# jojolebarjos/board-game-simulator-python

Measured on AMD Instinct MI355X. Metric: env-steps/sec, Connect4(6,7,4) random rollout, batch=2^20 per GPU, higher is better.
Workload: dtype u64

## Files before the change

### board-game-simulator-python_amd/csrc/connect_kernels.hip

```cpp
#include <type_traits>

#include "bgs_common.h"
#include "bgs_internal.h"
#include "connect_board.h"

#ifndef BGS_TU_ID
#define BGS_TU_ID "unknown"
#endif
extern "C" const char bgs_tu_id_connect[] = BGS_TU_ID;

namespace bgs {
namespace {

template <int NW_, int SH, int SW, int SK>
struct Geo {
    static constexpr int NW = NW_;
    static constexpr int STATIC_H = SH, STATIC_W = SW, STATIC_K = SK;
    static constexpr int MAXW = SW ? SW : BGS_CONNECT_MAX_W;
    int rh, rw, rk;
    __device__ __forceinline__ int h() const { return SH ? SH : rh; }
    __device__ __forceinline__ int w() const { return SW ? SW : rw; }
    __device__ __forceinline__ int k() const { return SK ? SK : rk; }
    __device__ __forceinline__ uint32_t all_columns() const { return (1u << w()) - 1u; }
};
// ... 733 lines not shown
        skip = 0;

        if (was_live != 0 && live == 0) {
            const uint32_t code = st ? st : (open == 0u ? BGS_ST_DRAW : BGS_ST_RUNNING);
            *reinterpret_cast<uint64_t*>(reinterpret_cast<char*>(plane0) + (game * 8u)) = p[0];
            *reinterpret_cast<uint64_t*>(reinterpret_cast<char*>(plane1) + (game * 8u)) = p[1];
            *(reinterpret_cast<uint8_t*>(status_out) + game) = (uint8_t)code;
            *reinterpret_cast<uint16_t*>(reinterpret_cast<char*>(reward_out) + (game * 2u)) = reward_pair(code);
            if (CODES) codes.add(game, code);
        }
    } while (__builtin_amdgcn_ballot_w64(live != 0) || taken < avail);
    if (CODES) codes.flush(codes_out, begin);
    add_steps(steps, stepped);
}

template <class G, int OPEN_BLOCKS, bool PER_PLY = false>
struct OpenedWords {
    static constexpr int LAST = G::STATIC_H > 0 ? (G::STATIC_H * G::STATIC_W + 3) / 4 - 1 : 11;
    static constexpr int COUNT = PER_PLY ? 1 : (LAST - OPEN_BLOCKS + 1 > 1 ? LAST - OPEN_BLOCKS + 1 : 1);
    static constexpr int QUADS = (COUNT + 3) / 4;
    static_assert(LAST <= 11 && OPEN_BLOCKS >= 1 && OPEN_BLOCKS <= 4, "three philox calls cover blocks 0 .. 11");
};

template <int QUADS>
struct OpenedPool {
    static constexpr uint32_t SLOTS = 64;
    uint64_t plane[2][SLOTS];
    uint32_t cols[SLOTS];
    uint4 words[QUADS][SLOTS];
};

constexpr uint32_t kReplayMark = 1u << 28;
constexpr uint32_t kReplayRow = 0x80000000u;

template <class G, int OPEN_BLOCKS, bool PER_PLY>
constexpr bool deferred_opening() {
    if constexpr (G::STATIC_H > 0 && G::STATIC_W > 0 && G::STATIC_K > 0)
        return !PER_PLY && kDeferredOpeningStages > 0 && OPEN_BLOCKS == kRolloutOpeningBlocks && kRolloutOpeningBlocks == 3 &&
               deferred_opening_ok(G::STATIC_H, G::STATIC_W, G::STATIC_K);
    else
        return false;
}

template <class G, class Pool>
__device__ __forceinline__ void open_games_deferred(const G& g, Pool& pool, uint32_t slot, uint64_t seed, uint64_t id, bool mine) {
    constexpr uint32_t ONES = 0x11111111u;
    const uint32_t top = (uint32_t)g.h() + 7u;
    const uint32_t columns = ONES & ((1u << (4 * g.w())) - 1u);
    const uint32_t stride = (uint32_t)g.h() + 1u;
    uint64_t q[2] = {0, 0};
    uint32_t h4 = top * columns;
    auto cheap_ply = [&](uint32_t j, uint32_t draw, bool wrap) {
        const uint32_t col = sample_index(draw, (uint32_t)g.w());
        const uint32_t sh = col * 4u;
        const uint32_t v = (h4 >> sh) & 15u;
        uint32_t pos = col * stride + top - v;
        if (wrap) pos &= 63u;
        q[j & 1u] |= 1ull << pos;
        h4 -= 1u << sh;
    };
    auto blind_block = [&](uint32_t word, bool wrap) -> bool {
        cheap_ply(0u, sub_draw<0>(word), wrap);
        cheap_ply(1u, sub_draw<1>(word), wrap);
        cheap_ply(2u, sub_draw<2>(word), wrap);
        const bool closed = ((h4 >> 3) & ONES) != columns;
        cheap_ply(3u, sub_draw<3>(word), wrap);
        return closed;
    };
    auto park = [&](uint32_t cols, const uint4& lo, const uint4& hi) {
        pool.plane[0][slot] = q[0];
        pool.plane[1][slot] = q[1];
        pool.cols[slot] = cols;
        pool.words[0][slot] = lo;
        pool.words[1][slot] = hi;
    };
    const Philox4 a = philox4x32_10(seed, id, 0u);
    cheap_ply(0u, sub_draw<0>(a.v[0]), false);
    cheap_ply(1u, sub_draw<1>(a.v[0]), false);
    cheap_ply(2u, sub_draw<2>(a.v[0]), false);
    cheap_ply(3u, sub_draw<3>(a.v[0]), false);
    uint32_t* const slot_words0 = reinterpret_cast<uint32_t*>(&pool.words[0][slot]);
    uint32_t* const slot_words1 = reinterpret_cast<uint32_t*>(&pool.words[1][slot]);
    slot_words0[0] = a.v[1]; slot_words0[1] = a.v[2]; slot_words0[2] = a.v[3];
    uint64_t id_after = id;
    asm volatile("" : "+v"(id_after) : : "memory");
    uint32_t word9, word10;
    {
        Philox4 c = philox4x32_10(seed, id_after, 2u);
        slot_words1[3] = c.v[0];
        word9 = c.v[1];
        word10 = c.v[2];
        asm volatile("" : "+v"(id_after), "+v"(word9), "+v"(word10) : : "memory");
    }
    {
        const Philox4 b = philox4x32_10(seed, id_after, 1u);
        slot_words0[3] = b.v[0];
        slot_words1[0] = b.v[1]; slot_words1[1] = b.v[2]; slot_words1[2] = b.v[3];
    }
    pool.plane[0][slot] = q[0];
    pool.plane[1][slot] = q[1];
    pool.cols[slot] = mine ? (h4 | kReplayMark) : 0u;
    asm volatile("" ::: "memory");
    blind_block(slot_words0[0], false);
    const bool closed = blind_block(slot_words0[1], false);
    const uint32_t hits = four_in_a_row_low_hits(q[0], g.h()) | four_in_a_row_low_hits(q[1], g.h());
    const bool clean = mine && !closed && hits == 0u;
    if (clean) {
        const uint4 lo = pool.words[0][slot], hi = pool.words[1][slot];
        park(h4, make_uint4(lo.z, lo.w, hi.x, hi.y), make_uint4(hi.z, hi.w, word9, word10));
    }
    if constexpr (kDeferredOpeningStages >= 2) {
        asm volatile("" ::: "memory");
        const bool closed2 = blind_block(slot_words0[0], true);
        const uint32_t hits2 = four_in_a_row_low_hits(q[0], g.h()) | four_in_a_row_low_hits(q[1], g.h());
        if (clean && !closed2 && hits2 == 0u) {
            const uint4 lo = pool.words[0][slot], hi = pool.words[1][slot];
            park(h4, make_uint4(lo.y, lo.z, lo.w, hi.x), make_uint4(hi.y, hi.z, hi.w, 0u));
        }
    }
}

template <class G, int OPEN_BLOCKS, bool CODES, bool PER_PLY>
__global__ void __launch_bounds__(BGS_BLOCK)
k_connect_rollout_opened(G g, uint64_t* __restrict__ planes, uint8_t* __restrict__ status, uint16_t* __restrict__ reward,
                         int64_t n, uint64_t seed, uint64_t first_game, unsigned long long* __restrict__ steps,
                         uint32_t games_per_wave, uint32_t* __restrict__ codes_out) {
    using OW = OpenedWords<G, OPEN_BLOCKS, PER_PLY>;
    constexpr int NWORDS = OW::QUADS * 4;
    using Pool = OpenedPool<OW::QUADS>;
    constexpr bool DEFER = deferred_opening<G, OPEN_BLOCKS, PER_PLY>();
    static_assert(!DEFER || NWORDS == 8, "a replayed game refills rows 5 .. 7 with the words of blocks 8 .. 10");
    extern __shared__ uint32_t code_lds[];
    __shared__ Pool pools[BGS_BLOCK / BGS_WAVE];
    __shared__ uint32_t lane_words[BGS_BLOCK / BGS_WAVE][NWORDS][BGS_WAVE];
    constexpr uint32_t ONES = 0x11111111u;
    const uint32_t top = (uint32_t)g.h() + 7u;
    const uint32_t columns = g.w() >= 8 ? ONES : (ONES & ((1u << (4 * g.w())) - 1u));
    const uint32_t stride = (uint32_t)g.h() + 1u;
    const uint32_t column_top = 8u * columns;
    const uint64_t eights = 0x88888888ull;

    const uint32_t wave = __builtin_amdgcn_readfirstlane(blockIdx.x * (BGS_BLOCK / BGS_WAVE) + (threadIdx.x >> 6));
    const uint32_t lane = threadIdx.x & 63u;
    const int64_t begin = (int64_t)wave * games_per_wave;
    const int64_t end = begin + games_per_wave < n ? begin + games_per_wave : n;
    const uint32_t avail = begin < end ? (uint32_t)(end - begin) : 0u;
    uint32_t taken = 0;
    uint32_t opened = 0;
    uint64_t* __restrict__ const plane0 = planes + begin;
    uint64_t* __restrict__ const plane1 = planes + n + begin;
    Pool& pool = pools[threadIdx.x >> 6];

    uint64_t p[2] = {0, 0};
    uint32_t hts = 0, live = 0, game = 0, stepped = 0;
    bool anywon = false;
    uint32_t wnext = 0;
    uint32_t* const my_words = &lane_words[threadIdx.x >> 6][0][lane];
    uint32_t wrow = 0;
    uint32_t myblk = 0;

    if (avail == 0u) return;
    uint8_t* const outcome = reinterpret_cast<uint8_t*>(code_lds + (threadIdx.x >> 6) * (games_per_wave >> 2));
    for (uint32_t i = lane; i < ((avail + 3u) >> 2); i += BGS_WAVE) reinterpret_cast<uint32_t*>(outcome)[i] = 0u;
    __builtin_amdgcn_wave_barrier();

    auto full_ply = [&](auto j_tag, uint32_t draw, uint64_t (&q)[2], uint32_t& h4, uint32_t& op, uint32_t& alive,
                        bool& won_any) {
        constexpr uint32_t J = decltype(j_tag)::value;
        const uint32_t cnt = (uint32_t)__popc(op);
        const uint32_t idx = sample_index(draw, cnt);
        uint64_t cmp64;
        {
            uint64_t carry;
            asm("v_mad_u64_u32 %0, %1, %2, %3, %4" : "=v"(cmp64), "=s"(carry) : "v"(idx - op), "s"(ONES), "v"(eights));
        }
        const uint32_t cmp = (uint32_t)cmp64;
        uint32_t col = (uint32_t)__popc(cmp & column_top);
        if (g.w() >= 8) col &= 7u;
        const uint32_t sh = col * 4u;
        const uint32_t v = (h4 >> sh) & 15u;
        uint32_t base = col * stride + top;
        asm("" : "+v"(base));
        uint32_t pos = base - v;
        if ((uint32_t)g.w() * stride + top > 63u) pos &= 63u;
        const uint32_t act = alive;
        uint64_t& mine = q[J & 1u];
        const uint64_t bit = 1ull << pos;
        mine = ((uint64_t)and_or((uint32_t)(bit >> 32), act, (uint32_t)(mine >> 32)) << 32) |
               and_or((uint32_t)bit, act, (uint32_t)mine);
        h4 += act << sh;
        op = (h4 >> 3) & ONES;
        bool won;
        if (g.k() == 4) {
            won = ply_run_of_four(g, mine, pos);
        } else {
            Bits<1> b;
            b.w[0] = mine;
            won = has_run(g, b);
        }
        won_any = won_any || won;
        alive = (won || op == 0u) ? 0u : alive;
    };
    auto outcome_of = [&](const uint64_t (&q)[2], bool won_any) -> uint32_t {
        const uint32_t stones = (uint32_t)__popcll(q[0]) + (uint32_t)__popcll(q[1]);
        stepped += stones;
        return won_any ? ((stones - 1u) & 1u) + 1u : (uint32_t)BGS_ST_DRAW;
    };
    auto cheap_ply = [&](uint32_t j, uint32_t draw, uint64_t (&q)[2], uint32_t& h4) {
        const uint32_t col = sample_index(draw, (uint32_t)g.w());
        const uint32_t sh = col * 4u;
        const uint32_t v = (h4 >> sh) & 15u;
        const uint32_t pos = col * stride + top - v;
        q[j & 1u] |= 1ull << pos;
        h4 -= 1u << sh;
    };
    auto refetch = [&](uint64_t lane_seed, uint64_t id) {
        if (wrow == (kReplayRow | 7u)) {
            if (live != 0u) {
                const Philox4 d = philox4x32_10(lane_seed, id, 2u);
                my_words[5 * BGS_WAVE] = d.v[0];
                my_words[6 * BGS_WAVE] = d.v[1];
                my_words[7 * BGS_WAVE] = d.v[2];
            }
            wrow = 5u;
        }
    };
    auto play_block = [&]() {
        const uint32_t was_live = live;
        Philox4 four = {{0u, 0u, 0u, 0u}};
        uint32_t word = 0u;
        if constexpr (PER_PLY) {
            four = philox4x32_10(seed, first_game + (uint64_t)(begin + game), myblk);
            myblk += 1u;
        } else if constexpr (DEFER) {
            word = wnext;
            if (__builtin_amdgcn_ballot_w64(wrow == (kReplayRow | 7u))) refetch(seed, first_game + (uint64_t)(begin + game));
            wnext = my_words[wrow * BGS_WAVE];
            const int32_t up = (int32_t)(wrow + 1u);
            wrow = (uint32_t)(up < NWORDS - 1 ? up : NWORDS - 1);
        } else {
            word = wnext;
            wnext = my_words[wrow * BGS_WAVE];
            wrow = wrow + 1u < (uint32_t)NWORDS - 1u ? wrow + 1u : (uint32_t)NWORDS - 1u;
        }
        uint32_t open = (hts >> 3) & ONES;
        full_ply(std::integral_constant<uint32_t, 0>{}, PER_PLY ? four.v[0] : sub_draw<0>(word), p, hts, open, live, anywon);
        full_ply(std::integral_constant<uint32_t, 1>{}, PER_PLY ? four.v[1] : sub_draw<1>(word), p, hts, open, live, anywon);
        full_ply(std::integral_constant<uint32_t, 2>{}, PER_PLY ? four.v[2] : sub_draw<2>(word), p, hts, open, live, anywon);
        full_ply(std::integral_constant<uint32_t, 3>{}, PER_PLY ? four.v[3] : sub_draw<3>(word), p, hts, open, live, anywon);
        if (was_live != 0 && live == 0) {
            *reinterpret_cast<uint64_t*>(reinterpret_cast<char*>(plane0) + (game * 8u)) = p[0];
            *reinterpret_cast<uint64_t*>(reinterpret_cast<char*>(plane1) + (game * 8u)) = p[1];
            outcome[game] = (uint8_t)outcome_of(p, anywon);
        }
    };
    auto take = [&](uint32_t which) {
        game = which;
        const uint32_t slot = which & (Pool::SLOTS - 1u);
        p[0] = pool.plane[0][slot];
        p[1] = pool.plane[1][slot];
        hts = pool.cols[slot];
        if constexpr (PER_PLY) {
            myblk = (uint32_t)OPEN_BLOCKS;
        } else {
#pragma unroll
            for (int k = 0; k < OW::QUADS; ++k) {
                const uint4 v = pool.words[k][slot];
                if (k == 0) wnext = v.x; else my_words[(4 * k) * BGS_WAVE] = v.x;
                my_words[(4 * k + 1) * BGS_WAVE] = v.y;
                my_words[(4 * k + 2) * BGS_WAVE] = v.z;
                my_words[(4 * k + 3) * BGS_WAVE] = v.w;
            }
        }
        wrow = DEFER ? 1u | ((hts << 3) & kReplayRow) : 1u;
        anywon = false;
        live = hts != 0u ? ~0u : 0u;
    };
    auto open_games = [&]() {
        const uint32_t og = opened + lane;
        const uint64_t id = first_game + (uint64_t)(begin + og);
        if constexpr (DEFER) {
            open_games_deferred(g, pool, og & (Pool::SLOTS - 1u), seed, id, og < avail);
            opened += 64u;
            return;
        }
        uint64_t q[2] = {0, 0};
        uint32_t h4 = top * columns, alive = ~0u, op = columns;
        bool won_any = false;
        uint32_t words[12];
        Philox4 own = philox4x32_10(seed, id, 0u);
        using J0 = std::integral_constant<uint32_t, 0>; using J1 = std::integral_constant<uint32_t, 1>;
        using J2 = std::integral_constant<uint32_t, 2>; using J3 = std::integral_constant<uint32_t, 3>;
#define BGS_DRAW_OF(JT, b) (PER_PLY ? own.v[JT::value] : sub_draw<JT::value>(words[b]))
        if constexpr (!PER_PLY) {
            words[0] = own.v[0]; words[1] = own.v[1]; words[2] = own.v[2]; words[3] = own.v[3];
#pragma unroll
            for (int c = 1; c < 3; ++c) {
                if (4 * c <= OW::LAST) {
                    const Philox4 d = philox4x32_10(seed, id, (uint32_t)c);
                    words[4 * c] = d.v[0]; words[4 * c + 1] = d.v[1]; words[4 * c + 2] = d.v[2]; words[4 * c + 3] = d.v[3];
                } else {
                    words[4 * c] = words[4 * c + 1] = words[4 * c + 2] = words[4 * c + 3] = 0u;
                }
            }
        } else {
#pragma unroll
            for (int c = 0; c < 12; ++c) words[c] = 0u;
        }
        cheap_ply(0u, BGS_DRAW_OF(J0, 0), q, h4);
        cheap_ply(1u, BGS_DRAW_OF(J1, 0), q, h4);
        cheap_ply(2u, BGS_DRAW_OF(J2, 0), q, h4);
        cheap_ply(3u, BGS_DRAW_OF(J3, 0), q, h4);
        if (OPEN_BLOCKS >= 2) {
            if constexpr (PER_PLY) own = philox4x32_10(seed, id, 1u);
            cheap_ply(0u, BGS_DRAW_OF(J0, 1), q, h4);
            cheap_ply(1u, BGS_DRAW_OF(J1, 1), q, h4);
            op = (h4 >> 3) & ONES;
            full_ply(J2{}, BGS_DRAW_OF(J2, 1), q, h4, op, alive, won_any);
            full_ply(J3{}, BGS_DRAW_OF(J3, 1), q, h4, op, alive, won_any);
        }
#pragma unroll
        for (int ob = 2; ob < OPEN_BLOCKS; ++ob) {
            if constexpr (PER_PLY) own = philox4x32_10(seed, id, (uint32_t)ob);
            full_ply(J0{}, BGS_DRAW_OF(J0, ob), q, h4, op, alive, won_any);
            full_ply(J1{}, BGS_DRAW_OF(J1, ob), q, h4, op, alive, won_any);
            full_ply(J2{}, BGS_DRAW_OF(J2, ob), q, h4, op, alive, won_any);
            full_ply(J3{}, BGS_DRAW_OF(J3, ob), q, h4, op, alive, won_any);
        }
#undef BGS_DRAW_OF
        if (OPEN_BLOCKS >= 2 && og < avail && alive == 0) {
            plane0[og] = q[0];
            plane1[og] = q[1];
            outcome[og] = (uint8_t)outcome_of(q, won_any);
        }
        const uint32_t slot = og & (Pool::SLOTS - 1u);
        pool.plane[0][slot] = q[0];
        pool.plane[1][slot] = q[1];
        pool.cols[slot] = alive ? h4 : 0u;
#pragma unroll
        for (int k = 0; k < OW::QUADS; ++k) {
            auto at = [&](int i) { return OPEN_BLOCKS + i <= 11 ? words[OPEN_BLOCKS + i <= 11 ? OPEN_BLOCKS + i : 11] : 0u; };
            pool.words[k][slot] = make_uint4(at(4 * k), at(4 * k + 1), at(4 * k + 2), at(4 * k + 3));
        }
        opened += 64u;
    };

    while (taken < avail) {
        const uint64_t need = __builtin_amdgcn_ballot_w64(live == 0);
        if (need) {
            const uint32_t wanted = (uint32_t)__popcll(need);
            const uint32_t rank = __builtin_amdgcn_mbcnt_hi((uint32_t)(need >> 32), __builtin_amdgcn_mbcnt_lo((uint32_t)need, 0u));
            const uint32_t have = opened - taken;
            if (wanted > have && opened < avail) {
                const bool first = live == 0 && rank < have;
                const bool second = live == 0 && !first;
                if (first && taken + rank < avail) take(taken + rank);
                __builtin_amdgcn_fence(__ATOMIC_ACQ_REL, "wavefront");
                __builtin_amdgcn_wave_barrier();
                open_games();
                __builtin_amdgcn_fence(__ATOMIC_ACQ_REL, "wavefront");
                __builtin_amdgcn_wave_barrier();
                if (second && taken + rank < avail) take(taken + rank);
            } else if (live == 0 && taken + rank < avail) {
                take(taken + rank);
            }
            taken = avail - taken < wanted ? avail : taken + wanted;
        }
        play_block();
    }
    while (__builtin_amdgcn_ballot_w64(live != 0)) play_block();

    __builtin_amdgcn_fence(__ATOMIC_ACQ_REL, "wavefront");
    __builtin_amdgcn_wave_barrier();
    uint8_t* __restrict__ const status_out = status + begin;
    uint16_t* __restrict__ const reward_out = reward + begin;
    uint8_t* __restrict__ const packed_out = reinterpret_cast<uint8_t*>(codes_out) + (begin >> 2);
    for (uint32_t g4 = lane * 4u; g4 < avail; g4 += BGS_WAVE * 4u) {
        const uint32_t four = reinterpret_cast<const uint32_t*>(outcome)[g4 >> 2];
        if (CODES) packed_out[g4 >> 2] = (uint8_t)((four & 3u) | ((four >> 6) & 0xCu) | ((four >> 12) & 0x30u) | ((four >> 18) & 0xC0u));
        if (g4 + 4u <= avail) {
            *reinterpret_cast<uint32_t*>(status_out + g4) = four;
            uint2 r;
            r.x = (uint32_t)reward_pair(four & 255u) | ((uint32_t)reward_pair((four >> 8) & 255u) << 16);
            r.y = (uint32_t)reward_pair((four >> 16) & 255u) | ((uint32_t)reward_pair(four >> 24) << 16);
            *reinterpret_cast<uint2*>(reward_out + g4) = r;
        } else {
            for (uint32_t k = 0; g4 + k < avail; ++k) {
                const uint32_t ck = (four >> (8u * k)) & 255u;
                status_out[g4 + k] = (uint8_t)ck;
                reward_out[g4 + k] = reward_pair(ck);
            }
        }
    }
    add_steps(steps, stepped);
}

template <class G, int OPEN_BLOCKS, bool CODES>
__global__ void __launch_bounds__(BGS_BLOCK)
k_connect_rollout_opened_steps(G g, const ConnectGroup tab, int64_t n, uint32_t games_per_wave) {
    using OW = OpenedWords<G, OPEN_BLOCKS, false>;
    constexpr int NWORDS = OW::QUADS * 4;
    using Pool = OpenedPool<OW::QUADS>;
    constexpr bool DEFER = deferred_opening<G, OPEN_BLOCKS, false>();
    static_assert(!DEFER || NWORDS == 8, "a replayed game refills rows 5 .. 7 with the words of blocks 8 .. 10");
    extern __shared__ uint32_t code_lds[];
    __shared__ Pool pools[BGS_BLOCK / BGS_WAVE];
    __shared__ uint32_t lane_words[BGS_BLOCK / BGS_WAVE][NWORDS][BGS_WAVE];
    constexpr uint32_t ONES = 0x11111111u;
    const uint32_t top = (uint32_t)g.h() + 7u;
    const uint32_t columns = g.w() >= 8 ? ONES : (ONES & ((1u << (4 * g.w())) - 1u));
    const uint32_t stride = (uint32_t)g.h() + 1u;
    const uint32_t column_top = 8u * columns;
    const uint64_t eights = 0x88888888ull;

    const uint32_t wave = __builtin_amdgcn_readfirstlane(blockIdx.x * (BGS_BLOCK / BGS_WAVE) + (threadIdx.x >> 6));
    const uint32_t lane = threadIdx.x & 63u;
    const int64_t begin = (int64_t)wave * games_per_wave;
    const int64_t end = begin + games_per_wave < n ? begin + games_per_wave : n;
    const uint32_t avail = begin < end ? (uint32_t)(end - begin) : 0u;
    const uint32_t nsteps = (uint32_t)tab.count;
    uint32_t taken = 0, opened = 0;
    Pool& pool = pools[threadIdx.x >> 6];

    uint32_t cur = 0;
    bool pending = false;
    uint64_t cur_seed = tab.step[0].seed, cur_first = tab.step[0].first_game;
    uint64_t* cur_planes = tab.step[0].planes ? tab.step[0].planes + begin : nullptr;
    uint64_t* prev_planes = nullptr;
    uint64_t prev_seed = 0, prev_first = 0;

    uint64_t p[2] = {0, 0};
    uint32_t hts = 0, live = 0, game = 0;
    uint32_t old = 0;
    uint32_t stepped0 = 0, stepped1 = 0;
    bool anywon = false;
    uint32_t wnext = 0;
    uint32_t* const my_words = &lane_words[threadIdx.x >> 6][0][lane];
    uint32_t wrow = 0;

    if (avail == 0u) return;
    uint8_t* const slices = reinterpret_cast<uint8_t*>(code_lds + (threadIdx.x >> 6) * (games_per_wave >> 1));
    auto slice_of = [&](uint32_t s) { return slices + (s & 1u) * games_per_wave; };
    auto zero_slice = [&](uint32_t s) {
        uint32_t* const w = reinterpret_cast<uint32_t*>(slice_of(s));
        for (uint32_t i = lane; i < ((avail + 3u) >> 2); i += BGS_WAVE) w[i] = 0u;
        __builtin_amdgcn_fence(__ATOMIC_ACQ_REL, "wavefront");
        __builtin_amdgcn_wave_barrier();
    };
    zero_slice(0u);

    auto full_ply = [&](auto j_tag, uint32_t draw, uint64_t (&q)[2], uint32_t& h4, uint32_t& op, uint32_t& alive,
                        bool& won_any) {
        constexpr uint32_t J = decltype(j_tag)::value;
        const uint32_t cnt = (uint32_t)__popc(op);
        const uint32_t idx = sample_index(draw, cnt);
        uint64_t cmp64;
        {
            uint64_t carry;
            asm("v_mad_u64_u32 %0, %1, %2, %3, %4" : "=v"(cmp64), "=s"(carry) : "v"(idx - op), "s"(ONES), "v"(eights));
        }
        const uint32_t cmp = (uint32_t)cmp64;
        uint32_t col = (uint32_t)__popc(cmp & column_top);
        if (g.w() >= 8) col &= 7u;
        const uint32_t sh = col * 4u;
        const uint32_t v = (h4 >> sh) & 15u;
        uint32_t base = col * stride + top;
        asm("" : "+v"(base));
        uint32_t pos = base - v;
        if ((uint32_t)g.w() * stride + top > 63u) pos &= 63u;
        const uint32_t act = alive;
        uint64_t& mine = q[J & 1u];
        const uint64_t bit = 1ull << pos;
        mine = ((uint64_t)and_or((uint32_t)(bit >> 32), act, (uint32_t)(mine >> 32)) << 32) |
               and_or((uint32_t)bit, act, (uint32_t)mine);
        h4 += act << sh;
        op = (h4 >> 3) & ONES;
        bool won;
        if (g.k() == 4) {
            won = ply_run_of_four(g, mine, pos);
        } else {
            Bits<1> b;
            b.w[0] = mine;
            won = has_run(g, b);
        }
        won_any = won_any || won;
        alive = (won || op == 0u) ? 0u : alive;
    };
    auto outcome_of = [&](const uint64_t (&q)[2], bool won_any, uint32_t parity) -> uint32_t {
        const uint32_t stones = (uint32_t)__popcll(q[0]) + (uint32_t)__popcll(q[1]);
        stepped0 += parity ? 0u : stones;
        stepped1 += parity ? stones : 0u;
        return won_any ? ((stones - 1u) & 1u) + 1u : (uint32_t)BGS_ST_DRAW;
    };
    auto cheap_ply = [&](uint32_t j, uint32_t draw, uint64_t (&q)[2], uint32_t& h4) {
        const uint32_t col = sample_index(draw, (uint32_t)g.w());
        const uint32_t sh = col * 4u;
        const uint32_t v = (h4 >> sh) & 15u;
        const uint32_t pos = col * stride + top - v;
        q[j & 1u] |= 1ull << pos;
        h4 -= 1u << sh;
    };
    auto refetch = [&]() {
        const bool at = wrow == (kReplayRow | 7u);
#pragma unroll
        for (uint32_t o = 0; o < 2u; ++o) {
            const bool here = at && live != 0u && old == o;
            if (__builtin_amdgcn_ballot_w64(here) == 0) continue;
            if (here) {
                const Philox4 d = philox4x32_10(o ? prev_seed : cur_seed, (o ? prev_first : cur_first) + (uint64_t)(begin + game), 2u);
                my_words[5 * BGS_WAVE] = d.v[0];
                my_words[6 * BGS_WAVE] = d.v[1];
                my_words[7 * BGS_WAVE] = d.v[2];
            }
        }
        if (at) wrow = 5u;
    };
    auto play_block = [&]() {
        const uint32_t was_live = live;
        const uint32_t word = wnext;
        if constexpr (DEFER) {
            if (__builtin_amdgcn_ballot_w64(wrow == (kReplayRow | 7u))) refetch();
            wnext = my_words[wrow * BGS_WAVE];
            const int32_t up = (int32_t)(wrow + 1u);
            wrow = (uint32_t)(up < NWORDS - 1 ? up : NWORDS - 1);
        } else {
            wnext = my_words[wrow * BGS_WAVE];
            wrow = wrow + 1u < (uint32_t)NWORDS - 1u ? wrow + 1u : (uint32_t)NWORDS - 1u;
        }
        uint32_t open = (hts >> 3) & ONES;
        full_ply(std::integral_constant<uint32_t, 0>{}, sub_draw<0>(word), p, hts, open, live, anywon);
        full_ply(std::integral_constant<uint32_t, 1>{}, sub_draw<1>(word), p, hts, open, live, anywon);
        full_ply(std::integral_constant<uint32_t, 2>{}, sub_draw<2>(word), p, hts, open, live, anywon);
        full_ply(std::integral_constant<uint32_t, 3>{}, sub_draw<3>(word), p, hts, open, live, anywon);
        if (was_live != 0 && live == 0) {
            uint64_t* const planes = old ? prev_planes : cur_planes;
            if (planes) {
                *reinterpret_cast<uint64_t*>(reinterpret_cast<char*>(planes) + (game * 8u)) = p[0];
                *reinterpret_cast<uint64_t*>(reinterpret_cast<char*>(planes + n) + (game * 8u)) = p[1];
            }
            const uint32_t s = cur - old;
            slice_of(s)[game] = (uint8_t)outcome_of(p, anywon, s & 1u);
        }
    };
    auto take = [&](uint32_t which) {
        game = which;
        old = 0u;
        const uint32_t slot = which & (Pool::SLOTS - 1u);
        p[0] = pool.plane[0][slot];
        p[1] = pool.plane[1][slot];
        hts = pool.cols[slot];
#pragma unroll
        for (int k = 0; k < OW::QUADS; ++k) {
            const uint4 v = pool.words[k][slot];
            if (k == 0) wnext = v.x; else my_words[(4 * k) * BGS_WAVE] = v.x;
            my_words[(4 * k + 1) * BGS_WAVE] = v.y;
            my_words[(4 * k + 2) * BGS_WAVE] = v.z;
            my_words[(4 * k + 3) * BGS_WAVE] = v.w;
        }
        wrow = DEFER ? 1u | ((hts << 3) & kReplayRow) : 1u;
        anywon = false;
        live = hts != 0u ? ~0u : 0u;
    };
    auto open_games = [&]() {
        const uint32_t og = opened + lane;
        const uint64_t id = cur_first + (uint64_t)(begin + og);
        if constexpr (DEFER) {
            open_games_deferred(g, pool, og & (Pool::SLOTS - 1u), cur_seed, id, og < avail);
            opened += 64u;
            return;
        }
        uint64_t q[2] = {0, 0};
        uint32_t h4 = top * columns, alive = ~0u, op = columns;
        bool won_any = false;
        uint32_t words[12];
        const Philox4 own = philox4x32_10(cur_seed, id, 0u);
        using J2 = std::integral_constant<uint32_t, 2>; using J3 = std::integral_constant<uint32_t, 3>;
        using J0 = std::integral_constant<uint32_t, 0>; using J1 = std::integral_constant<uint32_t, 1>;
        words[0] = own.v[0]; words[1] = own.v[1]; words[2] = own.v[2]; words[3] = own.v[3];
#pragma unroll
        for (int c = 1; c < 3; ++c) {
            if (4 * c <= OW::LAST) {
                const Philox4 d = philox4x32_10(cur_seed, id, (uint32_t)c);
                words[4 * c] = d.v[0]; words[4 * c + 1] = d.v[1]; words[4 * c + 2] = d.v[2]; words[4 * c + 3] = d.v[3];
            } else {
                words[4 * c] = words[4 * c + 1] = words[4 * c + 2] = words[4 * c + 3] = 0u;
            }
        }
        cheap_ply(0u, sub_draw<0>(words[0]), q, h4);
        cheap_ply(1u, sub_draw<1>(words[0]), q, h4);
        cheap_ply(2u, sub_draw<2>(words[0]), q, h4);
        cheap_ply(3u, sub_draw<3>(words[0]), q, h4);
        if (OPEN_BLOCKS >= 2) {
            cheap_ply(0u, sub_draw<0>(words[1]), q, h4);
            cheap_ply(1u, sub_draw<1>(words[1]), q, h4);
            op = (h4 >> 3) & ONES;
            full_ply(J2{}, sub_draw<2>(words[1]), q, h4, op, alive, won_any);
            full_ply(J3{}, sub_draw<3>(words[1]), q, h4, op, alive, won_any);
        }
#pragma unroll
        for (int ob = 2; ob < OPEN_BLOCKS; ++ob) {
            full_ply(J0{}, sub_draw<0>(words[ob]), q, h4, op, alive, won_any);
            full_ply(J1{}, sub_draw<1>(words[ob]), q, h4, op, alive, won_any);
            full_ply(J2{}, sub_draw<2>(words[ob]), q, h4, op, alive, won_any);
            full_ply(J3{}, sub_draw<3>(words[ob]), q, h4, op, alive, won_any);
        }
        if (OPEN_BLOCKS >= 2 && og < avail && alive == 0) {
            if (cur_planes) {
                cur_planes[og] = q[0];
                cur_planes[n + og] = q[1];
            }
            slice_of(cur)[og] = (uint8_t)outcome_of(q, won_any, cur & 1u);
        }
        const uint32_t slot = og & (Pool::SLOTS - 1u);
        pool.plane[0][slot] = q[0];
        pool.plane[1][slot] = q[1];
        pool.cols[slot] = alive ? h4 : 0u;
#pragma unroll
        for (int k = 0; k < OW::QUADS; ++k) {
            auto at = [&](int i) { return OPEN_BLOCKS + i <= 11 ? words[OPEN_BLOCKS + i <= 11 ? OPEN_BLOCKS + i : 11] : 0u; };
            pool.words[k][slot] = make_uint4(at(4 * k), at(4 * k + 1), at(4 * k + 2), at(4 * k + 3));
        }
        opened += 64u;
    };
    auto flush = [&](uint32_t s) {
        __builtin_amdgcn_fence(__ATOMIC_ACQ_REL, "wavefront");
        __builtin_amdgcn_wave_barrier();
        const ConnectGroupStep& e = tab.step[s];
        const uint8_t* const outcome = slice_of(s);
        if (e.planes) {
            uint8_t* __restrict__ const status_out = e.status + begin;
            uint16_t* __restrict__ const reward_out = e.reward + begin;
            for (uint32_t g4 = lane * 4u; g4 < avail; g4 += BGS_WAVE * 4u) {
                const uint32_t four = reinterpret_cast<const uint32_t*>(outcome)[g4 >> 2];
                if (g4 + 4u <= avail) {
                    *reinterpret_cast<uint32_t*>(status_out + g4) = four;
                    uint2 r;
                    r.x = (uint32_t)reward_pair(four & 255u) | ((uint32_t)reward_pair((four >> 8) & 255u) << 16);
                    r.y = (uint32_t)reward_pair((four >> 16) & 255u) | ((uint32_t)reward_pair(four >> 24) << 16);
                    *reinterpret_cast<uint2*>(reward_out + g4) = r;
                } else {
                    for (uint32_t k = 0; g4 + k < avail; ++k) {
                        const uint32_t ck = (four >> (8u * k)) & 255u;
                        status_out[g4 + k] = (uint8_t)ck;
                        reward_out[g4 + k] = reward_pair(ck);
                    }
                }
            }
        }
        if (CODES) {
            uint8_t* __restrict__ const packed_out = reinterpret_cast<uint8_t*>(e.codes) + (begin >> 2);
#pragma unroll 1
            for (uint32_t g4 = lane * 4u; g4 < avail; g4 += BGS_WAVE * 4u) {
                const uint32_t four = reinterpret_cast<const uint32_t*>(outcome)[g4 >> 2];
                packed_out[g4 >> 2] = (uint8_t)((four & 3u) | ((four >> 6) & 0xCu) | ((four >> 12) & 0x30u) | ((four >> 18) & 0xC0u));
            }
        }
        const uint32_t odd = s & 1u;
        add_steps(e.steps, odd ? stepped1 : stepped0);
        stepped0 = odd ? stepped0 : 0u;
        stepped1 = odd ? 0u : stepped1;
    };
    auto flush_done = [&]() {
        if (pending && __builtin_amdgcn_ballot_w64(live != 0 && old != 0) == 0) {
            flush(cur - 1u);
            pending = false;
        }
    };

    while (taken < avail || cur + 1u < nsteps) {
        const uint64_t need = __builtin_amdgcn_ballot_w64(live == 0);
        if (need) {
            const bool needy = live == 0;
            const uint32_t wanted = (uint32_t)__popcll(need);
            const uint32_t rank = __builtin_amdgcn_mbcnt_hi((uint32_t)(need >> 32), __builtin_amdgcn_mbcnt_lo((uint32_t)need, 0u));
            const uint32_t have = opened - taken;
            if (wanted > have && opened < avail) {
                const bool first = needy && rank < have;
                const bool second = needy && !first;
                if (first && taken + rank < avail) take(taken + rank);
                __builtin_amdgcn_fence(__ATOMIC_ACQ_REL, "wavefront");
                __builtin_amdgcn_wave_barrier();
                open_games();
                __builtin_amdgcn_fence(__ATOMIC_ACQ_REL, "wavefront");
                __builtin_amdgcn_wave_barrier();
                if (second && taken + rank < avail) take(taken + rank);
            } else if (needy && taken + rank < avail) {
                take(taken + rank);
            }
            const uint32_t served = avail - taken < wanted ? avail - taken : wanted;
            taken += served;
            if (served < wanted && cur + 1u < nsteps && !pending) {
                old = 1u;
                prev_planes = cur_planes;
                prev_seed = cur_seed;
                prev_first = cur_first;
                cur = __builtin_amdgcn_readfirstlane(cur + 1u);
                pending = true;
                cur_seed = tab.step[cur].seed;
                cur_first = tab.step[cur].first_game;
                cur_planes = tab.step[cur].planes ? tab.step[cur].planes + begin : nullptr;
                zero_slice(cur);
                taken = 0;
                opened = 0;
                open_games();
                __builtin_amdgcn_fence(__ATOMIC_ACQ_REL, "wavefront");
                __builtin_amdgcn_wave_barrier();
                if (needy && rank >= served && rank - served < avail) take(rank - served);
                taken = avail < wanted - served ? avail : wanted - served;
            }
        }
        play_block();
        flush_done();
    }
    while (__builtin_amdgcn_ballot_w64(live != 0)) {
        play_block();
        flush_done();
    }
    if (pending) flush(cur - 1u);
    flush(cur);
}

template <class G, bool CAPPED>
__global__ void __launch_bounds__(BGS_BLOCK)
k_connect_rollout_aligned_wide(G g, uint64_t* __restrict__ planes, uint8_t* __restrict__ status,
                               uint16_t* __restrict__ reward, int64_t n, uint64_t seed, uint64_t first_game,
                               uint32_t max_plies, unsigned long long* __restrict__ steps, uint32_t games_per_wave,
                               uint32_t per_ply) {
    constexpr int NW = G::NW;
    constexpr uint32_t ONES = 0x11111111u;
    const int h = g.h(), w = g.w();
    const uint32_t open_lo0 = w >= 8 ? ONES : (ONES & ((1u << (4 * w)) - 1u));
    const uint32_t open_hi0 = w <= 8 ? 0u : (w >= 16 ? ONES : (ONES & ((1u << (4 * (w - 8))) - 1u)));

    const uint32_t wave = __builtin_amdgcn_readfirstlane(blockIdx.x * (BGS_BLOCK / BGS_WAVE) + (threadIdx.x >> 6));
    const int64_t begin = (int64_t)wave * games_per_wave;
    const int64_t end = begin + games_per_wave < n ? begin + games_per_wave : n;
    const uint32_t avail = begin < end ? (uint32_t)(end - begin) : 0u;
    uint32_t taken = 0;

    Bits<NW> p[2] = {zero_bits<NW>(), zero_bits<NW>()};
    uint64_t hts = 0;
    uint32_t open_lo = 0, open_hi = 0;
    uint32_t blk = 0, st = 0, game = 0, stepped = 0;
    uint64_t live = 0;

    if (avail == 0u) return;
    do {
        const uint64_t need = __builtin_amdgcn_ballot_w64(live == 0);
        if (need && taken < avail) {
            const uint32_t rank = __builtin_amdgcn_mbcnt_hi((uint32_t)(need >> 32), __builtin_amdgcn_mbcnt_lo((uint32_t)need, 0u));
            if (live == 0 && taken + rank < avail) {
                game = taken + rank;
                p[0] = zero_bits<NW>();
                p[1] = zero_bits<NW>();
                hts = 0;
                open_lo = open_lo0;
                open_hi = open_hi0;
                blk = 0;
                st = 0;
                live = (!CAPPED || max_plies > 0u) ? 1u : 0u;
                if (CAPPED && live == 0) {
                    store_planes<NW>(planes, n, begin + game, p[0], p[1]);
                    status[begin + game] = 0;
                    reward[begin + game] = 0;
                }
            }
            const uint32_t wanted = (uint32_t)__popcll(need);
            taken = avail - taken < wanted ? avail : taken + wanted;
        }

        const uint64_t was_live = live;
        const Philox4 four = philox4x32_10(seed, first_game + (uint64_t)(begin + game), per_ply ? blk : blk >> 2);
        const uint32_t word = philox_word(four, blk);
#pragma unroll
        for (uint32_t j = 0; j < 4; ++j) {
            const uint32_t count_lo = (uint32_t)__popc(open_lo);
            const uint32_t idx = sample_index(per_ply ? four.v[j] : sub_draw(word, j), count_lo + (uint32_t)__popc(open_hi));
            const bool in_lo = idx < count_lo;
            const uint32_t part = in_lo ? open_lo : open_hi;
            const uint32_t rank_in_part = in_lo ? idx : idx - count_lo;
            const uint32_t cmp = (rank_in_part - part) * ONES + 0x88888888u;
            const uint32_t col = ((uint32_t)__popc(cmp & 0x88888888u) & 7u) + (in_lo ? 0u : 8u);
            const uint32_t v = (uint32_t)(hts >> (4u * col)) & 15u;
            const uint32_t pos = col * (uint32_t)(h + 1) + v;
            Bits<NW>& mine = p[j & 1u];
            const uint64_t stone = live << (pos & 63u);
#pragma unroll
            for (int i = 0; i < NW; ++i) mine.w[i] |= ((pos >> 6) == (uint32_t)i) ? stone : 0ull;
            hts += live << (4u * col);
            const uint32_t filled = (live != 0 && v + 1u == (uint32_t)h) ? (1u << (4u * (col & 7u))) : 0u;
            open_lo &= ~(in_lo ? filled : 0u);
            open_hi &= ~(in_lo ? 0u : filled);
            const bool won = has_run(g, mine);
            stepped += (uint32_t)live;
            st = (live != 0 && won) ? (j & 1u) + 1u : st;
            live = (won || (open_lo | open_hi) == 0u) ? 0 : live;
            if (CAPPED) live = (4u * blk + j + 1u < max_plies) ? live : 0;
        }
        blk += 1u;

        if (was_live != 0 && live == 0) {
            const int64_t i = begin + game;
            const uint32_t code = st ? st : ((open_lo | open_hi) == 0u ? BGS_ST_DRAW : BGS_ST_RUNNING);
            store_planes<NW>(planes, n, i, p[0], p[1]);
            status[i] = (uint8_t)code;
            reward[i] = reward_pair(code);
        }
    } while (__builtin_amdgcn_ballot_w64(live != 0) || taken < avail);
    add_steps(steps, stepped);
}

template <class G>
struct LdsBoard {
    static constexpr int H = G::STATIC_H, W = G::STATIC_W, K = G::STATIC_K;
    static constexpr int R = (K - 1) * (H + 2);
    static constexpr bool fits = H > 0 && K >= 2 && 2 * R <= 127;
    static constexpr int PB = (R + 31) / 32;
    static constexpr int PD = 2 * G::NW;
    static constexpr int ND = PB + PD + PB + 2;
    static constexpr size_t lds_bytes = (size_t)2 * ND * BGS_BLOCK * sizeof(uint32_t);
};

struct Win {
    uint32_t d[4];
};

template <int C>
__device__ __forceinline__ Win win_shr(const Win& x) {
    constexpr int q = C >> 5, r = C & 31;
    Win y;
#pragma unroll
    for (int i = 0; i < 4; ++i) {
        const uint32_t lo = (i + q < 4) ? x.d[(i + q) & 3] : 0u;
        const uint32_t hi = (i + q + 1 < 4) ? x.d[(i + q + 1) & 3] : 0u;
        y.d[i] = r ? __builtin_amdgcn_alignbit(hi, lo, r) : lo;
    }
    return y;
}

__device__ __forceinline__ Win win_and(const Win& a, const Win& b) {
    Win y;
#pragma unroll
    for (int i = 0; i < 4; ++i) y.d[i] = a.d[i] & b.d[i];
    return y;
}

template <int D, int LEN, int K>
__device__ __forceinline__ Win win_runs(const Win& m) {
    if constexpr (LEN >= K) {
// ... 815 lines not shown
```

### board-game-simulator-python_amd/csrc/connect_unit.h

```cpp
#pragma once

#include <stdint.h>

struct ConnectGeom {
    int h, w, k, nw;
};

constexpr int kRolloutOpeningBlocks = 3;
constexpr int kGamesPerLaneOneWord = 8;
constexpr int kGamesPerLane = 4;

constexpr bool runs_start_low(int h, int w) { return (w - 4) * (h + 1) + h - 1 <= 31; }

constexpr bool deferred_opening_ok(int h, int w, int k) {
    return k == 4 && w >= 4 && w <= 7 && h <= 8 && w * (h + 1) <= 64 && runs_start_low(h, w) && 2 * k - 1 > 4 && h > 4 &&
           h + 7 >= 12 && h * w <= 44;
}
constexpr int kDeferredOpeningStages = 2;

constexpr int kConnectGroupSteps = 2;
constexpr int kConnectGroupMax = 8;
constexpr int kConnectGroupMinCall = 48;

struct ConnectGroupStep {
    uint64_t seed;
    uint64_t first_game;
    uint64_t* planes;
    uint8_t* status;
    uint16_t* reward;
    uint32_t* codes;
    unsigned long long* steps;
};
struct ConnectGroup {
    ConnectGroupStep step[kConnectGroupMax];
    int count;
};
```

Measured before the change: 974.9 billion.

## Encode ply count in outcome bytes and derive status, reward, steps in SWAR flush

Outcome bytes now store the stone count plus a run flag instead of the final status code. Status, reward, packed codes and step counts are then decoded four games at a time with SWAR arithmetic during the flush. This removes the per-game stepped accumulators from the hot play loop and merges the codes and status loops into one pass. The grouped kernel also switches to absolute slice offsets in LDS, which adds index arithmetic for plane writes and replay seeding.

After: 1011 billion (median of 6 runs). 3.7% higher.

```diff
diff --git a/board-game-simulator-python_amd/csrc/connect_kernels.hip b/board-game-simulator-python_amd/csrc/connect_kernels.hip
--- a/board-game-simulator-python_amd/csrc/connect_kernels.hip
+++ b/board-game-simulator-python_amd/csrc/connect_kernels.hip
@@ -909,7 +909,7 @@
     Pool& pool = pools[threadIdx.x >> 6];
 
     uint64_t p[2] = {0, 0};
-    uint32_t hts = 0, live = 0, game = 0, stepped = 0;
+    uint32_t hts = 0, live = 0, game = 0;
     bool anywon = false;
     uint32_t wnext = 0;
     uint32_t* const my_words = &lane_words[threadIdx.x >> 6][0][lane];
@@ -960,8 +960,7 @@
     };
     auto outcome_of = [&](const uint64_t (&q)[2], bool won_any) -> uint32_t {
         const uint32_t stones = (uint32_t)__popcll(q[0]) + (uint32_t)__popcll(q[1]);
-        stepped += stones;
-        return won_any ? ((stones - 1u) & 1u) + 1u : (uint32_t)BGS_ST_DRAW;
+        return connect_outcome_byte(stones, won_any);
     };
     auto cheap_ply = [&](uint32_t j, uint32_t draw, uint64_t (&q)[2], uint32_t& h4) {
         const uint32_t col = sample_index(draw, (uint32_t)g.w());
@@ -1132,20 +1131,18 @@
     uint8_t* __restrict__ const status_out = status + begin;
     uint16_t* __restrict__ const reward_out = reward + begin;
     uint8_t* __restrict__ const packed_out = reinterpret_cast<uint8_t*>(codes_out) + (begin >> 2);
+    uint32_t stepped = 0;
     for (uint32_t g4 = lane * 4u; g4 < avail; g4 += BGS_WAVE * 4u) {
-        const uint32_t four = reinterpret_cast<const uint32_t*>(outcome)[g4 >> 2];
-        if (CODES) packed_out[g4 >> 2] = (uint8_t)((four & 3u) | ((four >> 6) & 0xCu) | ((four >> 12) & 0x30u) | ((four >> 18) & 0xC0u));
+        const ConnectOutcome4 o = connect_outcome4(reinterpret_cast<const uint32_t*>(outcome)[g4 >> 2]);
+        stepped += o.plies;
+        if (CODES) packed_out[g4 >> 2] = (uint8_t)o.codes;
         if (g4 + 4u <= avail) {
-            *reinterpret_cast<uint32_t*>(status_out + g4) = four;
-            uint2 r;
-            r.x = (uint32_t)reward_pair(four & 255u) | ((uint32_t)reward_pair((four >> 8) & 255u) << 16);
-            r.y = (uint32_t)reward_pair((four >> 16) & 255u) | ((uint32_t)reward_pair(four >> 24) << 16);
-            *reinterpret_cast<uint2*>(reward_out + g4) = r;
+            *reinterpret_cast<uint32_t*>(status_out + g4) = o.status;
+            *reinterpret_cast<uint2*>(reward_out + g4) = make_uint2(o.reward[0], o.reward[1]);
         } else {
             for (uint32_t k = 0; g4 + k < avail; ++k) {
-                const uint32_t ck = (four >> (8u * k)) & 255u;
-                status_out[g4 + k] = (uint8_t)ck;
-                reward_out[g4 + k] = reward_pair(ck);
+                status_out[g4 + k] = (uint8_t)(o.status >> (8u * k));
+                reward_out[g4 + k] = (uint16_t)((((uint64_t)o.reward[1] << 32) | o.reward[0]) >> (16u * k));
             }
         }
     }
@@ -1187,17 +1184,20 @@
     uint64_t prev_seed = 0, prev_first = 0;
 
     uint64_t p[2] = {0, 0};
-    uint32_t hts = 0, live = 0, game = 0;
+    uint32_t hts = 0, live = 0;
+    uint32_t game = 0;
     uint32_t old = 0;
-    uint32_t stepped0 = 0, stepped1 = 0;
     bool anywon = false;
     uint32_t wnext = 0;
     uint32_t* const my_words = &lane_words[threadIdx.x >> 6][0][lane];
     uint32_t wrow = 0;
 
     if (avail == 0u) return;
-    uint8_t* const slices = reinterpret_cast<uint8_t*>(code_lds + (threadIdx.x >> 6) * (games_per_wave >> 1));
-    auto slice_of = [&](uint32_t s) { return slices + (s & 1u) * games_per_wave; };
+    uint8_t* const outcome_bytes = reinterpret_cast<uint8_t*>(code_lds);
+    const uint32_t slices_at = __builtin_amdgcn_readfirstlane((threadIdx.x >> 6) * 2u * games_per_wave);
+    auto slice_at = [&](uint32_t s) { return slices_at + (s & 1u) * games_per_wave; };
+    auto slice_of = [&](uint32_t s) { return outcome_bytes + slice_at(s); };
+    uint32_t cur_at = slice_at(0u), prev_at = 0;
     auto zero_slice = [&](uint32_t s) {
         uint32_t* const w = reinterpret_cast<uint32_t*>(slice_of(s));
         for (uint32_t i = lane; i < ((avail + 3u) >> 2); i += BGS_WAVE) w[i] = 0u;
@@ -1243,11 +1243,9 @@
         won_any = won_any || won;
         alive = (won || op == 0u) ? 0u : alive;
     };
-    auto outcome_of = [&](const uint64_t (&q)[2], bool won_any, uint32_t parity) -> uint32_t {
+    auto outcome_of = [&](const uint64_t (&q)[2], bool won_any) -> uint32_t {
         const uint32_t stones = (uint32_t)__popcll(q[0]) + (uint32_t)__popcll(q[1]);
-        stepped0 += parity ? 0u : stones;
-        stepped1 += parity ? stones : 0u;
-        return won_any ? ((stones - 1u) & 1u) + 1u : (uint32_t)BGS_ST_DRAW;
+        return connect_outcome_byte(stones, won_any);
     };
     auto cheap_ply = [&](uint32_t j, uint32_t draw, uint64_t (&q)[2], uint32_t& h4) {
         const uint32_t col = sample_index(draw, (uint32_t)g.w());
@@ -1264,7 +1262,8 @@
             const bool here = at && live != 0u && old == o;
             if (__builtin_amdgcn_ballot_w64(here) == 0) continue;
             if (here) {
-                const Philox4 d = philox4x32_10(o ? prev_seed : cur_seed, (o ? prev_first : cur_first) + (uint64_t)(begin + game), 2u);
+                const Philox4 d = philox4x32_10(o ? prev_seed : cur_seed,
+                                                (o ? prev_first : cur_first) + (uint64_t)(begin + (game - (o ? prev_at : cur_at))), 2u);
                 my_words[5 * BGS_WAVE] = d.v[0];
                 my_words[6 * BGS_WAVE] = d.v[1];
                 my_words[7 * BGS_WAVE] = d.v[2];
@@ -1290,17 +1289,19 @@
         full_ply(std::integral_constant<uint32_t, 2>{}, sub_draw<2>(word), p, hts, open, live, anywon);
         full_ply(std::integral_constant<uint32_t, 3>{}, sub_draw<3>(word), p, hts, open, live, anywon);
         if (was_live != 0 && live == 0) {
-            uint64_t* const planes = old ? prev_planes : cur_planes;
-            if (planes) {
-                *reinterpret_cast<uint64_t*>(reinterpret_cast<char*>(planes) + (game * 8u)) = p[0];
-                *reinterpret_cast<uint64_t*>(reinterpret_cast<char*>(planes + n) + (game * 8u)) = p[1];
-            }
-            const uint32_t s = cur - old;
-            slice_of(s)[game] = (uint8_t)outcome_of(p, anywon, s & 1u);
+            if (cur_planes != nullptr || prev_planes != nullptr) {
+                uint64_t* const planes = old ? prev_planes : cur_planes;
+                if (planes) {
+                    const uint32_t at = (game - (old ? prev_at : cur_at)) * 8u;
+                    *reinterpret_cast<uint64_t*>(reinterpret_cast<char*>(planes) + at) = p[0];
+                    *reinterpret_cast<uint64_t*>(reinterpret_cast<char*>(planes + n) + at) = p[1];
+                }
+            }
+            outcome_bytes[game] = (uint8_t)outcome_of(p, anywon);
         }
     };
     auto take = [&](uint32_t which) {
-        game = which;
+        game = cur_at + which;
         old = 0u;
         const uint32_t slot = which & (Pool::SLOTS - 1u);
         p[0] = pool.plane[0][slot];
@@ -1366,7 +1367,7 @@
                 cur_planes[og] = q[0];
                 cur_planes[n + og] = q[1];
             }
-            slice_of(cur)[og] = (uint8_t)outcome_of(q, won_any, cur & 1u);
+            slice_of(cur)[og] = (uint8_t)outcome_of(q, won_any);
         }
         const uint32_t slot = og & (Pool::SLOTS - 1u);
         pool.plane[0][slot] = q[0];
@@ -1383,44 +1384,35 @@
         __builtin_amdgcn_fence(__ATOMIC_ACQ_REL, "wavefront");
         __builtin_amdgcn_wave_barrier();
         const ConnectGroupStep& e = tab.step[s];
-        const uint8_t* const outcome = slice_of(s);
-        if (e.planes) {
-            uint8_t* __restrict__ const status_out = e.status + begin;
-            uint16_t* __restrict__ const reward_out = e.reward + begin;
-            for (uint32_t g4 = lane * 4u; g4 < avail; g4 += BGS_WAVE * 4u) {
-                const uint32_t four = reinterpret_cast<const uint32_t*>(outcome)[g4 >> 2];
+        const uint32_t* const outcome = reinterpret_cast<const uint32_t*>(slice_of(s));
+        uint8_t* __restrict__ const status_out = e.status + begin;
+        uint16_t* __restrict__ const reward_out = e.reward + begin;
+        uint8_t* __restrict__ const packed_out = reinterpret_cast<uint8_t*>(e.codes) + (begin >> 2);
+        uint32_t stepped = 0;
+#pragma unroll 1
+        for (uint32_t g4 = lane * 4u; g4 < avail; g4 += BGS_WAVE * 4u) {
+            const ConnectOutcome4 o = connect_outcome4(outcome[g4 >> 2]);
+            stepped += o.plies;
+            if (CODES) packed_out[g4 >> 2] = (uint8_t)o.codes;
+            if (e.planes) {
                 if (g4 + 4u <= avail) {
-                    *reinterpret_cast<uint32_t*>(status_out + g4) = four;
-                    uint2 r;
-                    r.x = (uint32_t)reward_pair(four & 255u) | ((uint32_t)reward_pair((four >> 8) & 255u) << 16);
-                    r.y = (uint32_t)reward_pair((four >> 16) & 255u) | ((uint32_t)reward_pair(four >> 24) << 16);
-                    *reinterpret_cast<uint2*>(reward_out + g4) = r;
+                    *reinterpret_cast<uint32_t*>(status_out + g4) = o.status;
+                    *reinterpret_cast<uint2*>(reward_out + g4) = make_uint2(o.reward[0], o.reward[1]);
                 } else {
                     for (uint32_t k = 0; g4 + k < avail; ++k) {
-                        const uint32_t ck = (four >> (8u * k)) & 255u;
-                        status_out[g4 + k] = (uint8_t)ck;
-                        reward_out[g4 + k] = reward_pair(ck);
+                        status_out[g4 + k] = (uint8_t)(o.status >> (8u * k));
+                        reward_out[g4 + k] = (uint16_t)((((uint64_t)o.reward[1] << 32) | o.reward[0]) >> (16u * k));
                     }
                 }
             }
         }
-        if (CODES) {
-            uint8_t* __restrict__ const packed_out = reinterpret_cast<uint8_t*>(e.codes) + (begin >> 2);
-#pragma unroll 1
-            for (uint32_t g4 = lane * 4u; g4 < avail; g4 += BGS_WAVE * 4u) {
-                const uint32_t four = reinterpret_cast<const uint32_t*>(outcome)[g4 >> 2];
-                packed_out[g4 >> 2] = (uint8_t)((four & 3u) | ((four >> 6) & 0xCu) | ((four >> 12) & 0x30u) | ((four >> 18) & 0xC0u));
-            }
-        }
-        const uint32_t odd = s & 1u;
-        add_steps(e.steps, odd ? stepped1 : stepped0);
-        stepped0 = odd ? stepped0 : 0u;
-        stepped1 = odd ? 0u : stepped1;
+        add_steps(e.steps, stepped);
     };
     auto flush_done = [&]() {
         if (pending && __builtin_amdgcn_ballot_w64(live != 0 && old != 0) == 0) {
             flush(cur - 1u);
             pending = false;
+            prev_planes = nullptr;
         }
     };
 
@@ -1451,7 +1443,9 @@
                 prev_planes = cur_planes;
                 prev_seed = cur_seed;
                 prev_first = cur_first;
+                prev_at = cur_at;
                 cur = __builtin_amdgcn_readfirstlane(cur + 1u);
+                cur_at = slice_at(cur);
                 pending = true;
                 cur_seed = tab.step[cur].seed;
                 cur_first = tab.step[cur].first_game;
diff --git a/board-game-simulator-python_amd/csrc/connect_unit.h b/board-game-simulator-python_amd/csrc/connect_unit.h
--- a/board-game-simulator-python_amd/csrc/connect_unit.h
+++ b/board-game-simulator-python_amd/csrc/connect_unit.h
@@ -18,6 +18,37 @@
 }
 constexpr int kDeferredOpeningStages = 2;
 
+constexpr uint32_t kOutcomeRun = 64u;
+constexpr uint32_t connect_outcome_byte(uint32_t stones, bool run) { return stones | (run ? kOutcomeRun : 0u); }
+struct ConnectOutcome4 {
+    uint32_t status;
+    uint32_t reward[2];
+    uint32_t codes;
+    uint32_t plies;
+};
+constexpr ConnectOutcome4 connect_outcome4(uint32_t four) {
+    constexpr uint32_t L = 0x01010101u;
+    const uint32_t run = (four >> 6) & L, odd = four & L;
+    const uint32_t game = ((four + 0x7F7F7F7Fu) >> 7) & L;
+    const uint32_t low = game & ~(run & ~odd);
+    const uint32_t high = game & ~(run & odd);
+    const uint32_t status = low | (high << 1);
+    const uint32_t won1 = low & ~high, won2 = high & ~low;
+    const uint32_t a = (won1 & 1u) | ((won1 & 0x100u) << 8), b = (won2 & 1u) | ((won2 & 0x100u) << 8);
+    const uint32_t c = ((won1 >> 16) & 1u) | ((won1 >> 8) & 0x10000u), d = ((won2 >> 16) & 1u) | ((won2 >> 8) & 0x10000u);
+    return ConnectOutcome4{status,
+                           {a * 0xFF01u | b * 0x01FFu, c * 0xFF01u | d * 0x01FFu},
+                           (status & 3u) | ((status >> 6) & 0xCu) | ((status >> 12) & 0x30u) | ((status >> 18) & 0xC0u),
+                           ((four & 0x3F3F3F3Fu) * L) >> 24};
+}
+struct ConnectOutcome {
+    uint32_t status, reward, code, plies;
+};
+constexpr ConnectOutcome connect_outcome(uint32_t byte) {
+    const ConnectOutcome4 o = connect_outcome4(byte & 255u);
+    return ConnectOutcome{o.status, o.reward[0], o.codes, o.plies};
+}
+
 constexpr int kConnectGroupSteps = 2;
 constexpr int kConnectGroupMax = 8;
 constexpr int kConnectGroupMinCall = 48;
```
